# cs4247/music-transcription

Measured on AMD Instinct MI355X. Metric: 30 s audio chunks/sec (mel+CNNRNN forward), higher is better.
Workload: dtype f16; 1 GPU; CNNRNNModel inference, batch=32x30 s synthetic 16 kHz audio, mel+CNN-RNN HIP path (BASELINE.json configs[1]); batch_per_gpu=32, frames=938, coscheduled_batches_per_forward=4, streams_per_gpu=4, batches_in_flight=16, parallelism=dp1 (independent chunks)

## Files before the change

### include/mt_hip.h

```cpp
#ifndef MT_HIP_H
#define MT_HIP_H

#include <stddef.h>
#include <stdint.h>

#ifdef __cplusplus
extern "C" {
#endif

#define MT_OK            0
#define MT_EINVAL       -1
#define MT_EWORKSPACE   -2
#define MT_EHIP         -3
#define MT_EUNSUPPORTED -4

#define MT_DT_BF16 0
#define MT_DT_F16  1
#define MT_GX_F16  0x10

#define MT_N_FFT 2048
#define MT_N_PITCH 88

typedef void* mt_stream_t;

int         mt_version(void);
const char* mt_last_error(void);
int         mt_device_count(void);
int         mt_init(int device);
#define MT_WS_LSTM_GX        1
#define MT_WS_LSTM_HX        2
#define MT_WS_LSTM_CX        3
#define MT_WS_LSTM_SYNC      4
#define MT_WS_LSTM_BWD_PART  5
#define MT_WS_LSTM_DGX       6
#define MT_WS_MEL_PLAN       7
#define MT_WS_ADAM           8
size_t      mt_workspace_bytes(int kind, int B, int T, int H);
#define MT_AR_F32   0
#define MT_AR_BF16  1
#define MT_AR_F16   2
int         mt_allreduce(void* buf, size_t count, int dtype, void* comm, mt_stream_t stream);


int    mt_mel_filterbank_host(float* fb_host, int sr, int n_mels);
int    mt_mel_num_frames(int n_samples, int hop);

typedef struct { int sr, hop, n_mels, ell_rows; } mt_mel_desc;
size_t mt_mel_plan_bytes(int n_mels);
int    mt_mel_plan_init(void* plan, size_t plan_bytes, int sr, int hop, int n_mels, mt_mel_desc* desc,
                        mt_stream_t stream);

int    mt_mel_db_f32(const void* plan, const mt_mel_desc* desc, const float* wave, int B, int n_samples,
                     float* mel_db, float* chunk_max_power, int apply_clamp, mt_stream_t stream);

int    mt_mel_db_windows_f32(const void* plan, const mt_mel_desc* desc, const float* store, const long long* win_off,
                             const int* win_len, const int* rec_end, int B, int max_win_len, int T_out,
                             const int* t_keep, float* mel_db, float* chunk_max_power, mt_stream_t stream);

int    mt_roll_windows(const int* spans, const long long* pitch_off, const int* cols, const int* win_rec,
                       const long long* win_cols, const int* win_ncols, const int* t_keep, int B, int T_out,
                       float* roll, mt_stream_t stream);

int    mt_stitch_windows(const float* src, int Bw, int P, int Tw, const int* dst_row, const long long* dst_frame0,
                         const int* keep_lo, const int* keep_hi, float* dst, int R, long long T_dst, mt_stream_t stream);

int    mt_conv1_bn_relu_pool(const float* mel, const float* chunk_max_power, const float* w, const float* bias,
                             void* act1, int B, int n_mels, int T, mt_stream_t stream);
int    mt_conv2_bn_relu_pool(const void* act1, const void* w2, const float* bias, void* X0, int ldx,
                             int B, int F1, int T, mt_stream_t stream);
int    mt_conv1_bn_relu_pool_dt(const float* mel, const float* chunk_max_power, const float* w, const float* bias,
                                void* act1, int B, int n_mels, int T, int dt, mt_stream_t stream);
int    mt_conv12_bn_relu_pool_dt(const float* mel, const float* chunk_max_power, const float* w1, const float* b1,
                                 const void* w2, const float* b2, void* X0, int ldx, int B, int n_mels, int T, int dt,
                                 mt_stream_t stream);
int    mt_conv2_bn_relu_pool_dt(const void* act1, const void* w2, const float* bias, void* X0, int ldx,
                                int B, int F1, int T, int dt, mt_stream_t stream);

int    mt_gemm_bf16_f32acc(const void* A, int lda, const void* W, int ldw, const float* bias,
                           float* C, int ldc, int M, int N, int K, mt_stream_t stream);
int    mt_gemm_lstm_gx(const void* X, int ldx, const void* W_ih, int ldw, const float* bias, float* gx,
                       int B, int T, int H, int K, mt_stream_t stream);
int    mt_gemm_logits(const void* X, int ldx, const void* W, int ldw, const float* bias, float* logits,
                      int B, int T, int N, int K, mt_stream_t stream);
int    mt_gemm_lstm_gx_from_hx(const float* hx_prev, const void* W_ih, int ldw, const float* bias, float* gx,
                               int B, int T, int H, int Hprev, mt_stream_t stream);
int    mt_gemm_lstm_gx_from_hx_ex(const float* hx_prev, const void* W_ih, int ldw, const float* bias, float* gx,
                                  int B, int T, int H, int Hprev, int gx_f16, mt_stream_t stream);
int    mt_gemm_logits_from_hx(const float* hx_prev, const void* W, int ldw, const float* bias, float* logits,
                              int B, int T, int N, int Hprev, mt_stream_t stream);
int    mt_gemm_f32acc_dt(const void* A, int lda, const void* W, int ldw, const float* bias,
                         float* C, int ldc, int M, int N, int K, int dt, mt_stream_t stream);
int    mt_gemm_lstm_gx_dt(const void* X, int ldx, const void* W_ih, int ldw, const float* bias, float* gx,
                          int B, int T, int H, int K, int dt, mt_stream_t stream);
int    mt_gemm_logits_dt(const void* X, int ldx, const void* W, int ldw, const float* bias, float* logits,
                         int B, int T, int N, int K, int dt, mt_stream_t stream);
#define MT_GEMM_SCHED_BYTES 64
size_t mt_gemm_sched_bytes(void);
int    mt_gemm_lstm_gx_sched(const void* X, int ldx, const void* W_ih, int ldw, const float* bias, float* gx,
                             int B, int T, int H, int K, int dt, void* sched, mt_stream_t stream);
int    mt_gemm_lstm_gx_from_hx_sched(const float* hx_prev, const void* W_ih, int ldw, const float* bias, float* gx,
                                     int B, int T, int H, int Hprev, int gx_f16, void* sched, mt_stream_t stream);

size_t mt_lstm_gx_bytes(int B, int T, int H);
size_t mt_lstm_hx_bytes(int B, int T, int H);
size_t mt_lstm_sync_bytes(int B, int H);
int    mt_lstm_bidir_fwd(const float* gx, const float* w_hh, float* hx, void* sync_ws, size_t sync_bytes,
                         int B, int T, int H, mt_stream_t stream);
int    mt_lstm_bidir_fwd_xproj(const float* hx_prev, const float* w_ihx, const float* bias, const float* w_hh, float* hx,
                               void* sync_ws, size_t sync_bytes, int B, int T, int H, mt_stream_t stream);
int    mt_lstm_bidir_fwd_ex(const float* gx, const float* w_hh, float* hx, void* sync_ws, size_t sync_bytes,
                            int B, int T, int H, int flags, mt_stream_t stream);
int    mt_persistent_cus_in_flight(mt_stream_t stream);
int    mt_lstm_relayout_bf16(const float* hx, void* X, int ldx, int B, int T, int H, mt_stream_t stream);
int    mt_lstm_unpack_f32(const float* hx, float* y, int B, int T, int H, mt_stream_t stream);

#define MT_MAX_LSTM_LAYERS 8
typedef struct {
    int n_mels;
    int hidden;
    int layers;
    int operand_dtype;
    const float* conv1_w;
    const float* conv1_b;
    const void*  conv2_w;
    const float* conv2_b;
    const void*  w_ih[MT_MAX_LSTM_LAYERS];
    const float* b_gates[MT_MAX_LSTM_LAYERS];
    const float* w_hh[MT_MAX_LSTM_LAYERS];
    const void*  fc_w;
    const float* fc_b;
    const float* w_ihx[MT_MAX_LSTM_LAYERS];
} mt_cnnrnn_weights;

size_t mt_cnnrnn_workspace_bytes(const mt_cnnrnn_weights* w, int B, int T);
int    mt_cnnrnn_conv_fused(void);
size_t mt_cnnrnn_status_offset(const mt_cnnrnn_weights* w, int B, int T, int layer);
int    mt_cnnrnn_forward(const mt_cnnrnn_weights* w, const float* mel, const float* chunk_max_power,
                         int B, int T, float* logits, void* workspace, size_t workspace_bytes,
                         mt_stream_t stream);
int    mt_cnnrnn_num_stages(int layers);
int    mt_cnnrnn_forward_ex(const mt_cnnrnn_weights* w, const float* mel, const float* chunk_max_power,
                            int B, int T, float* logits, void* workspace, size_t workspace_bytes,
                            void* const* events, int n_events, mt_stream_t stream);

int    mt_conv_cl_bf16(const void* A, const void* S, const void* W, const float* bias, void* out,
                       int B, int F, int T, int C1, int C2, int Cout, int KH, int relu, int pool,
                       int out_mode, int ldx, mt_stream_t stream);
int    mt_gemm_batched_f32(const void* A, int lda, long long sA1, long long sA2, const void* W, int ldw,
                           long long sW1, long long sW2, const float* bias, float* C, int ldc,
                           long long sC1, long long sC2, int M, int N, int K, int batch, int zdiv,
                           mt_stream_t stream);
int    mt_gemm_batched_bf16out(const void* A, int lda, long long sA1, long long sA2, const void* W, int ldw,
                               long long sW1, long long sW2, const float* bias, void* C, int ldc,
                               long long sC1, long long sC2, int M, int N, int K, int batch, int zdiv,
// ... 245 lines not shown
```

### music-transcription_amd/_lib.py

```python
from __future__ import annotations

import ctypes as C
import os

_HERE = os.path.dirname(os.path.abspath(__file__))
LIB_PATH = os.path.join(_HERE, "libmt_hip.so")
MAX_LSTM_LAYERS = 8
N_PITCH = 88
DT_BF16, DT_F16 = 0, 1
GX_F16 = 0x10


class MtError(RuntimeError):
    pass


def build(verbose: bool = False) -> str:
    import subprocess
    r = subprocess.run(["make", "-C", os.path.join(_HERE, "csrc"), "-j8"], capture_output=True, text=True)
    if verbose or r.returncode != 0:
        print(r.stdout[-4000:], r.stderr[-4000:])
    if r.returncode != 0:
        raise MtError("building libmt_hip.so failed")
    return LIB_PATH


if not os.path.exists(LIB_PATH):
    raise ImportError(f"{LIB_PATH} not found: build it with `python -c 'import __graft_entry__ as g; g.build()'` "
                      f"or `make -C {os.path.join(_HERE, 'csrc')}` (needs hipcc)")

import torch as _torch

lib = C.CDLL(LIB_PATH)

vp, sz, i32, f32p = C.c_void_p, C.c_size_t, C.c_int, C.c_void_p


class MelDesc(C.Structure):
    _fields_ = [("sr", i32), ("hop", i32), ("n_mels", i32), ("ell_rows", i32)]


class CnnRnnWeights(C.Structure):
    _fields_ = [("n_mels", i32), ("hidden", i32), ("layers", i32), ("operand_dtype", i32),
                ("conv1_w", vp), ("conv1_b", vp), ("conv2_w", vp), ("conv2_b", vp),
                ("w_ih", vp * MAX_LSTM_LAYERS), ("b_gates", vp * MAX_LSTM_LAYERS), ("w_hh", vp * MAX_LSTM_LAYERS),
                ("fc_w", vp), ("fc_b", vp), ("w_ihx", vp * MAX_LSTM_LAYERS)]


class CnnRnnLargeWeights(C.Structure):
    _fields_ = ([(n, i32) for n in ("n_mels", "hidden", "layers", "hidden_local", "use_attention", "use_heads", "heads", "head_dim_pad")]
                + [("attn_scale", C.c_float), ("operand_dtype", i32)]
                + [(n, vp) for n in ("conv1_w", "conv1_b", "rb1c1_w", "rb1c1_b", "rb1c2_w", "rb1c2_b", "rb2c1_w", "rb2c1_b",
                                     "rb2c2_w", "rb2c2_b", "fa_w", "fa_b")]
                + [("main_w_ih", vp * MAX_LSTM_LAYERS), ("main_b", vp * MAX_LSTM_LAYERS), ("main_w_hh", vp * MAX_LSTM_LAYERS)]
                + [(n, vp) for n in ("local_w_ih", "local_b", "local_w_hh", "qkv_w", "qkv_b", "proj_w", "proj_b", "ln_g", "ln_b",
                                     "shared_w", "shared_b", "heads_w", "heads_b", "fc_w", "fc_b")]
                + [("main_w_ihx", vp * MAX_LSTM_LAYERS)])


ll = C.c_longlong
_SIGS = {
    "mt_version": (i32, []),
    "mt_last_error": (C.c_char_p, []),
    "mt_device_count": (i32, []),
    "mt_init": (i32, [i32]),
    "mt_workspace_bytes": (sz, [i32, i32, i32, i32]),
    "mt_allreduce": (i32, [vp, sz, i32, vp, vp]),
    "mt_mel_filterbank_host": (i32, [vp, i32, i32]),
    "mt_mel_num_frames": (i32, [i32, i32]),
    "mt_mel_plan_bytes": (sz, [i32]),
    "mt_mel_plan_init": (i32, [vp, sz, i32, i32, i32, C.POINTER(MelDesc), vp]),
    "mt_mel_db_f32": (i32, [vp, C.POINTER(MelDesc), vp, i32, i32, vp, vp, i32, vp]),
    "mt_mel_db_windows_f32": (i32, [vp, C.POINTER(MelDesc), vp, vp, vp, vp, i32, i32, i32, vp, vp, vp, vp]),
    "mt_roll_windows": (i32, [vp, vp, vp, vp, vp, vp, vp, i32, i32, vp, vp]),
    "mt_stitch_windows": (i32, [vp, i32, i32, i32, vp, vp, vp, vp, vp, i32, ll, vp]),
    "mt_conv1_bn_relu_pool": (i32, [vp, vp, vp, vp, vp, i32, i32, i32, vp]),
    "mt_conv2_bn_relu_pool": (i32, [vp, vp, vp, vp, i32, i32, i32, i32, vp]),
    "mt_conv1_bn_relu_pool_dt": (i32, [vp, vp, vp, vp, vp, i32, i32, i32, i32, vp]),
    "mt_conv2_bn_relu_pool_dt": (i32, [vp, vp, vp, vp, i32, i32, i32, i32, i32, vp]),
    "mt_cnnrnn_conv_fused": (i32, []),
    "mt_conv12_bn_relu_pool_dt": (i32, [vp, vp, vp, vp, vp, vp, vp, i32, i32, i32, i32, i32, vp]),
    "mt_gemm_f32acc_dt": (i32, [vp, i32, vp, i32, vp, vp, i32, i32, i32, i32, i32, vp]),
    "mt_gemm_lstm_gx_dt": (i32, [vp, i32, vp, i32, vp, vp, i32, i32, i32, i32, i32, vp]),
    "mt_gemm_logits_dt": (i32, [vp, i32, vp, i32, vp, vp, i32, i32, i32, i32, i32, vp]),
    "mt_conv_cl_dt": (i32, [vp, vp, vp, vp, vp] + [i32] * 12 + [vp]),
    "mt_gemm_batched_f32_dt": (i32, [vp, i32, ll, ll, vp, i32, ll, ll, vp, vp, i32, ll, ll, i32, i32, i32, i32, i32, i32, vp]),
    "mt_gemm_batched_h16out_dt": (i32, [vp, i32, ll, ll, vp, i32, ll, ll, vp, vp, i32, ll, ll, i32, i32, i32, i32, i32, i32, i32, vp]),
    "mt_lstm_relayout_dt": (i32, [vp, vp, i32, vp, i32, i32, i32, i32, i32, i32, i32, vp]),
    "mt_attn_softmax_clamped_dt": (i32, [vp, i32, vp, i32, i32, ll, C.c_float, C.c_float, i32, vp]),
    "mt_layernorm_residual_dt": (i32, [vp, i32, vp, i32, vp, vp, vp, i32, ll, i32, C.c_float, i32, vp]),
    "mt_gemm_lstm_gx_from_hx": (i32, [vp, vp, i32, vp, vp, i32, i32, i32, i32, vp]),
    "mt_gemm_lstm_gx_from_hx_ex": (i32, [vp, vp, i32, vp, vp, i32, i32, i32, i32, i32, vp]),
    "mt_gemm_logits_from_hx": (i32, [vp, vp, i32, vp, vp, i32, i32, i32, i32, vp]),
    "mt_gemm_bf16_f32acc": (i32, [vp, i32, vp, i32, vp, vp, i32, i32, i32, i32, vp]),
    "mt_gemm_lstm_gx": (i32, [vp, i32, vp, i32, vp, vp, i32, i32, i32, i32, vp]),
    "mt_gemm_sched_bytes": (sz, []),
    "mt_gemm_lstm_gx_sched": (i32, [vp, i32, vp, i32, vp, vp, i32, i32, i32, i32, i32, vp, vp]),
    "mt_gemm_lstm_gx_from_hx_sched": (i32, [vp, vp, i32, vp, vp, i32, i32, i32, i32, i32, vp, vp]),
    "mt_gemm_lstm_dh": (i32, [vp, i32, vp, i32, vp, i32, i32, i32, i32, i32, C.c_float, C.c_uint, C.c_uint, vp]),
    "mt_gemm_logits": (i32, [vp, i32, vp, i32, vp, vp, i32, i32, i32, i32, vp]),
    "mt_lstm_gx_bytes": (sz, [i32, i32, i32]),
    "mt_lstm_hx_bytes": (sz, [i32, i32, i32]),
    "mt_lstm_sync_bytes": (sz, [i32, i32]),
    "mt_lstm_bidir_fwd": (i32, [vp, vp, vp, vp, sz, i32, i32, i32, vp]),
    "mt_lstm_bidir_fwd_xproj": (i32, [vp, vp, vp, vp, vp, vp, sz, i32, i32, i32, vp]),
    "mt_lstm_bidir_fwd_ex": (i32, [vp, vp, vp, vp, sz, i32, i32, i32, i32, vp]),
    "mt_persistent_cus_in_flight": (i32, [vp]),
    "mt_lstm_relayout_bf16": (i32, [vp, vp, i32, i32, i32, i32, vp]),
    "mt_lstm_unpack_f32": (i32, [vp, vp, i32, i32, i32, vp]),
    "mt_conv_cl_bf16": (i32, [vp, vp, vp, vp, vp] + [i32] * 11 + [vp]),
    "mt_gemm_batched_f32": (i32, [vp, i32, ll, ll, vp, i32, ll, ll, vp, vp, i32, ll, ll, i32, i32, i32, i32, i32, vp]),
    "mt_gemm_batched_bf16out": (i32, [vp, i32, ll, ll, vp, i32, ll, ll, vp, vp, i32, ll, ll, i32, i32, i32, i32, i32, i32, vp]),
    "mt_lstm_relayout_ex": (i32, [vp, vp, i32, vp, i32, i32, i32, i32, i32, i32, vp]),
    "mt_attn_softmax_clamped": (i32, [vp, i32, vp, i32, i32, ll, C.c_float, C.c_float, vp]),
    "mt_attn_transpose_v": (i32, [vp, i32, i32, vp, i32, i32, i32, i32, i32, vp]),
    "mt_attn_fused_clamped": (i32, [vp, i32, i32, vp, i32, i32, i32, i32, i32, C.c_float, C.c_float, vp, i32, i32, vp]),
    "mt_layernorm_residual": (i32, [vp, i32, vp, i32, vp, vp, vp, i32, ll, i32, C.c_float, vp]),
    "mt_cnnrnn_large_workspace_bytes": (sz, [C.POINTER(CnnRnnLargeWeights), i32, i32]),
    "mt_cnnrnn_large_status_offset": (sz, [C.POINTER(CnnRnnLargeWeights), i32, i32, i32]),
    "mt_cnnrnn_large_forward": (i32, [C.POINTER(CnnRnnLargeWeights), vp, vp, i32, i32, vp, vp, sz, vp]),
    "mt_cnnrnn_large_forward_ex": (i32, [C.POINTER(CnnRnnLargeWeights), vp, vp, i32, i32, vp, vp, sz, vp, vp, vp, vp]),
    "mt_cnnrnn_large_num_stages": (i32, [i32]),
    "mt_cnnrnn_large_forward_ev": (i32, [C.POINTER(CnnRnnLargeWeights), vp, vp, i32, i32, vp, vp, sz, C.POINTER(vp), i32, vp]),
    "mt_adam_workspace_bytes": (sz, []),
    "mt_adam_clip_step": (i32, [vp, vp, vp, vp, ll] + [C.c_float] * 6 + [i32, vp, vp, sz, vp]),
    "mt_adam_clip_step_ex": (i32, [vp, vp, vp, vp, ll] + [C.c_float] * 6 + [i32, C.c_float, vp, i32, vp, vp, sz, vp]),
    "mt_bce_workspace_bytes": (sz, []),
    "mt_bce_masked_fwd_bwd": (i32, [vp, vp, vp, C.c_longlong, C.c_float, i32, vp, vp, vp, sz, i32, i32, i32, vp]),
    "mt_onset_offset_targets": (i32, [vp, vp, vp, C.c_longlong, i32, vp]),
    "mt_predict_threshold": (i32, [vp, vp, C.c_longlong, C.c_float, vp]),
    "mt_f1_counts": (i32, [vp, vp, vp, vp, i32, i32, i32, vp]),
    "mt_f1_sweep_counts": (i32, [vp, vp, vp, vp, i32, vp, i32, i32, i32, vp]),
    "mt_roll_to_notes": (i32, [vp, i32, C.c_float, i32, i32, i32, vp, vp, vp, i32, vp]),
    "mt_note_match_counts": (i32, [vp, vp, C.c_float, C.c_float, vp, vp, vp, i32, i32, i32, vp]),
    "mt_note_match_list": (i32, [vp, vp, C.c_float, C.c_float, vp, vp, vp, vp, vp, i32, i32, i32, vp]),
    "mt_note_sweep_counts": (i32, [vp, vp, vp, i32, vp, i32, vp, vp, vp, i32, i32, i32, vp]),
    "mt_note_sweep_list": (i32, [vp, vp, vp, i32, vp, i32, vp, vp, vp, vp, vp, i32, i32, i32, vp]),
    "mt_heads_to_notes": (i32, [vp, vp, C.c_float, C.c_float, i32, i32, i32, vp, vp, vp, i32, vp]),
    "mt_note_match_counts_off": (i32, [vp, vp, vp, C.c_float, C.c_float, C.c_float, vp, vp, vp, i32, i32, i32, vp]),
    "mt_note_match_list_off": (i32, [vp, vp, vp, C.c_float, C.c_float, C.c_float, vp, vp, vp, vp, vp, i32, i32, i32, vp]),
    "mt_heads_to_notes_off": (i32, [vp, vp, vp, C.c_float, C.c_float, C.c_float, i32, i32, i32, vp, vp, vp, i32, vp]),
    "mt_notes_batch": (i32, [vp, vp, C.c_float, C.c_float, vp, i32, i32, ll, vp, vp, vp, vp, ll, vp]),
    "mt_note_match_counts_clean": (i32, [vp, vp, vp, C.c_float, C.c_float, C.c_float, vp, vp, vp, i32, i32, i32, i32, i32, vp]),
    "mt_note_match_list_clean": (i32, [vp, vp, vp, C.c_float, C.c_float, C.c_float, vp, vp, vp, vp, vp, i32, i32, i32, i32, i32, vp]),
    "mt_heads_to_notes_clean": (i32, [vp, vp, vp, C.c_float, C.c_float, C.c_float, i32, i32, i32, vp, vp, vp, i32, i32, i32, vp]),
    "mt_notes_batch_clean": (i32, [vp, vp, C.c_float, C.c_float, vp, i32, i32, ll, vp, vp, vp, vp, ll, i32, i32, vp]),
    "mt_conv1_stats": (i32, [vp, vp, vp, vp, i32, i32, i32, vp]),
    "mt_bn_finalize": (i32, [vp, C.c_double, vp, vp, vp, vp, C.c_float, C.c_float, vp, vp, i32, vp, vp, vp, vp, i32, vp]),
    "mt_bn_stats_cl": (i32, [vp, ll, i32, vp, vp]),
    "mt_bn_relu_pool_apply": (i32, [vp, vp, vp, vp, vp, vp, i32, i32, i32, i32, vp]),
    "mt_bn_pool_bwd": (i32, [vp, i32, vp, vp, vp, vp, vp, vp, vp, vp, vp, vp, i32, i32, i32, vp]),
    "mt_conv_cl_tie": (i32, [vp, vp, vp, vp, vp, i32, i32, i32, i32, i32, i32, vp]),
    "mt_bn_pool_bwd_tie": (i32, [vp, i32, vp, vp, vp, vp, vp, vp, vp, vp, vp, vp, vp, i32, i32, i32, vp]),
    "mt_conv2_wgrad_workgroups": (i32, []),
    "mt_conv2_wgrad": (i32, [vp, vp, vp, vp, vp, i32, i32, i32, i32, vp]),
    "mt_pack_wih_cf": (i32, [vp, vp, ll, i32, i32, i32, i32, i32, i32, vp]),
    "mt_pack_jobs": (i32, [vp, i32, i32, vp]),
    "mt_transpose_bf16": (i32, [vp, ll, ll, i32, vp, ll, i32, vp]),
    "mt_gather4_f32": (i32, [vp, vp, i32, i32, i32, i32, ll, ll, ll, ll, C.c_float, vp]),
    "mt_sum_slices_f32": (i32, [vp, ll, i32, i32, vp, i32, i32, i32, vp]),
    "mt_rowsum_bf16": (i32, [vp, ll, ll, vp, i32, vp]),
    "mt_conv1_bwd": (i32, [vp] * 8 + [i32] + [vp] * 5 + [i32, i32, i32, vp]),
# ... 64 lines not shown
```

### music-transcription_amd/csrc/conv.hip

```cpp
#include "mt_common.h"

namespace mt {

template <int DT>
__global__ __launch_bounds__(256) void conv1_kernel(const float* __restrict__ mel, const unsigned* __restrict__ chunk_max,
                                                    const float* __restrict__ w , const float* __restrict__ bias ,
                                                    bf16_t* __restrict__ act1, int F, int T, int Fo) {
    const int t = blockIdx.x * 64 + (threadIdx.x & 63);
    const int fo = blockIdx.y * 4 + (threadIdx.x >> 6);
    const int b = blockIdx.z;
    if (t >= T || fo >= Fo) return;
    float floor_db = -3.0e38f;
    if (chunk_max) floor_db = 10.0f * log10f(fmaxf(__uint_as_float(chunk_max[b]), 1e-10f)) - 80.0f;
    const float* m = mel + (size_t)b * F * T;
    float p[4][3];
#pragma unroll
    for (int r = 0; r < 4; ++r) {
        const int f = 2 * fo - 1 + r;
#pragma unroll
        for (int c = 0; c < 3; ++c) {
            const int tt = t - 1 + c;
            const bool in = (f >= 0 && f < F && tt >= 0 && tt < T);
            p[r][c] = in ? fmaxf(m[(size_t)f * T + tt], floor_db) : 0.0f;
        }
    }
    typedef float f2_t __attribute__((ext_vector_type(2)));
    f2_t pp[3][3][1];
#pragma unroll
    for (int kh = 0; kh < 3; ++kh)
#pragma unroll
        for (int kw = 0; kw < 3; ++kw) pp[kh][kw][0] = f2_t{p[kh][kw], p[kh + 1][kw]};
    unsigned packed[16];
#pragma unroll
    for (int c = 0; c < 32; ++c) {
        f2_t a = f2_t{bias[c], bias[c]};
#pragma unroll
        for (int kh = 0; kh < 3; ++kh)
#pragma unroll
            for (int kw = 0; kw < 3; ++kw) {
                const float wv = w[c * 9 + kh * 3 + kw];
                a = __builtin_elementwise_fma(f2_t{wv, wv}, pp[kh][kw][0], a);
            }
        const float v = fmaxf(fmaxf(a.x, a.y), 0.0f);
        if (c & 1) packed[c >> 1] |= ((unsigned)f32_to_h16<DT>(v)) << 16;
        else packed[c >> 1] = f32_to_h16<DT>(v);
    }
    uint4* dst = (uint4*)(act1 + (((size_t)b * Fo + fo) * T + t) * 32);
#pragma unroll
    for (int i = 0; i < 4; ++i) dst[i] = make_uint4(packed[4 * i], packed[4 * i + 1], packed[4 * i + 2], packed[4 * i + 3]);
}

constexpr int C2_TF = 16, C2_TT = 16;
constexpr int C2_ROWS = 2 * C2_TF + 2, C2_PITCH = 20;

constexpr int C2_DMA_INSTRS = (C2_ROWS * C2_PITCH * 4 + 63) / 64;
constexpr int C2_LDS_BYTES = C2_DMA_INSTRS * 1024;

template <int DT>
__global__ __launch_bounds__(256, 2) void conv2_kernel(const bf16_t* __restrict__ act1, const bf16_t* __restrict__ w2 ,
                                                       const float* __restrict__ bias , bf16_t* __restrict__ X0,
                                                       int B, int F1, int T, int Fo2, int ldx, int tiles_f, int tiles_t) {
    extern __shared__ __attribute__((aligned(16))) char in_s[];
    const int tid = threadIdx.x, wv = tid >> 6, lane = tid & 63;
    const int ntile = wv & 1, mgrp = wv >> 1;
    const int r = lane & 31, h = lane >> 5;
    const int t_l = r & 15, fbit = r >> 4;
    const int co = ntile * 32 + r;
    const float bv = bias[co];
    bf16x8 wf[18];
#pragma unroll
    for (int ks = 0; ks < 18; ++ks) wf[ks] = *(const bf16x8*)(w2 + (size_t)co * 288 + ks * 16 + h * 8);

    const int n_tiles = B * tiles_f * tiles_t;
    typedef __attribute__((address_space(3))) void lvoid_t;
#define C2_ISSUE_DMA(TILE)                                                                                     \
    do {                                                                                                       \
        const int tile_ = (TILE);                                                                              \
        if (tile_ < n_tiles) {                                                                                 \
            const int b_ = tile_ / (tiles_f * tiles_t), rem_ = tile_ - b_ * tiles_f * tiles_t;                 \
            const int fy_ = rem_ / tiles_t, tx_ = rem_ - fy_ * tiles_t;                                        \
            const int fb_ = 2 * fy_ * C2_TF - 1, tb_ = tx_ * C2_TT - 1;                                        \
            const __amdgpu_buffer_rsrc_t rs_ = __builtin_amdgcn_make_buffer_rsrc(                              \
                (void*)(act1 + (size_t)b_ * F1 * T * 32), 0, F1 * T * 64, 0x00020000);                         \
            for (int q_ = wv; q_ < C2_DMA_INSTRS; q_ += 4) {                                                   \
                const int p_ = q_ * 64 + lane, pos_ = p_ >> 2, slot_ = p_ & 3;                                 \
                const int row_ = pos_ / C2_PITCH, col_ = pos_ - row_ * C2_PITCH;                               \
                const int f_ = fb_ + row_, t_ = tb_ + col_;                                                    \
                const bool ok_ = row_ < C2_ROWS && col_ < 18 && f_ >= 0 && f_ < F1 && t_ >= 0 && t_ < T;       \
                const int off_ = ok_ ? ((f_ * T + t_) * 64 + ((slot_ ^ ((col_ >> 2) & 3)) << 4)) : 0x7fffffff; \
                __builtin_amdgcn_raw_ptr_buffer_load_lds(rs_, (lvoid_t*)(in_s + q_ * 1024), 16, off_, 0, 0, 0); \
            }                                                                                                  \
        }                                                                                                      \
    } while (0)

    C2_ISSUE_DMA(blockIdx.x);
    for (int tile = blockIdx.x; tile < n_tiles; tile += gridDim.x) {
        const int b = tile / (tiles_f * tiles_t), rem = tile - b * tiles_f * tiles_t;
        const int fy = rem / tiles_t, tx = rem - fy * tiles_t;
        const int t0 = tx * C2_TT, fo0 = fy * C2_TF;
        asm volatile("s_waitcnt vmcnt(0)" ::: "memory");
        __builtin_amdgcn_s_barrier();
#pragma unroll 1
        for (int half = 0; half < 2; ++half) {
            f32x16 acc[4];
#pragma unroll
            for (int i = 0; i < 4; ++i)
#pragma unroll
                for (int j = 0; j < 16; ++j) acc[i][j] = 0.0f;
#pragma unroll
            for (int tap = 0; tap < 9; ++tap) {
                const int kh = tap / 3, kw = tap % 3;
                const int col = t_l + kw;
#pragma unroll
                for (int s2 = 0; s2 < 2; ++s2) {
                    const int chunk = (s2 * 2 + h) ^ ((col >> 2) & 3);
#pragma unroll
                    for (int mi = 0; mi < 4; ++mi) {
                        const int row = 2 * (mgrp * 8 + half * 4 + mi) + fbit + kh;
                        const bf16x8 afrag = *(const bf16x8*)(in_s + (row * C2_PITCH + col) * 64 + (chunk << 4));
                        acc[mi] = mfma_32x32x16<DT>(afrag, wf[tap * 2 + s2], acc[mi]);
                    }
                }
            }
            if (half == 1) {
                asm volatile("s_waitcnt lgkmcnt(0)" ::: "memory");
                __builtin_amdgcn_s_barrier();
                C2_ISSUE_DMA(tile + gridDim.x);
            }
#pragma unroll
            for (int mi = 0; mi < 4; ++mi) {
                const int fo = fo0 + mgrp * 8 + half * 4 + mi;
                if (fo >= Fo2) continue;
#pragma unroll
                for (int q = 0; q < 2; ++q)
#pragma unroll
                    for (int p = 0; p < 4; ++p) {
                        const int tl = p + 8 * q + 4 * h, t = t0 + tl;
                        const float v = fmaxf(fmaxf(acc[mi][4 * q + p], acc[mi][4 * (q + 2) + p]) + bv, 0.0f);
                        if (t < T) X0[((size_t)t * B + b) * ldx + fo * 64 + co] = f32_to_h16<DT>(v);
                    }
            }
        }
    }
#undef C2_ISSUE_DMA
}

constexpr int C12_MROWS = 2 * C2_ROWS + 2, C12_MCOLS = 20, C12_MPITCH = 21;
constexpr int C12_MEL_ELEMS = C12_MROWS * C12_MCOLS;
constexpr int C12_MEL_PER_THREAD = (C12_MEL_ELEMS + 255) / 256;
constexpr int C12_POS = C2_ROWS * 18;
constexpr int C12_LDS_BYTES = C2_LDS_BYTES + C12_MROWS * C12_MPITCH * 4;

template <int DT>
__global__ __launch_bounds__(256, 2) void conv12_kernel(const float* __restrict__ mel, const unsigned* __restrict__ chunk_max,
                                                        const float* __restrict__ w1 , const float* __restrict__ b1 ,
                                                        const bf16_t* __restrict__ w2 , const float* __restrict__ bias ,
                                                        bf16_t* __restrict__ X0, int B, int F, int F1, int T, int Fo2, int ldx, int tiles_f,
                                                        int tiles_t) {
    extern __shared__ __attribute__((aligned(16))) char in_s[];
    float* ms = (float*)(in_s + C2_LDS_BYTES);
    const int tid = threadIdx.x, wv = tid >> 6, lane = tid & 63;
    const int ntile = wv & 1, mgrp = wv >> 1;
    const int r = lane & 31, h = lane >> 5;
    const int t_l = r & 15, fbit = r >> 4;
    const int co = ntile * 32 + r;
    const float bv = bias[co];
    bf16x8 wf[18];
#pragma unroll
    for (int ks = 0; ks < 18; ++ks) wf[ks] = *(const bf16x8*)(w2 + (size_t)co * 288 + ks * 16 + h * 8);
    const int n_tiles = B * tiles_f * tiles_t;

    float mreg[C12_MEL_PER_THREAD];
    auto load_mel = [&](int tile_) {
        if (tile_ >= n_tiles) return;
        const int b_ = tile_ / (tiles_f * tiles_t), rem_ = tile_ - b_ * tiles_f * tiles_t;
        const int fy_ = rem_ / tiles_t, tx_ = rem_ - fy_ * tiles_t;
        const int m0_ = 2 * (2 * fy_ * C2_TF - 1) - 1, tc0_ = tx_ * C2_TT - 2;
        float floor_db = -3.0e38f;
        if (chunk_max) floor_db = 10.0f * log10f(fmaxf(__uint_as_float(chunk_max[b_]), 1e-10f)) - 80.0f;
        const float* m = mel + (size_t)b_ * F * T;
#pragma unroll
        for (int k = 0; k < C12_MEL_PER_THREAD; ++k) {
            const int idx = tid + 256 * k, lr = idx / C12_MCOLS, lc = idx - lr * C12_MCOLS;
            const int f = m0_ + lr, tt = tc0_ + lc;
            const bool in = idx < C12_MEL_ELEMS && f >= 0 && f < F && tt >= 0 && tt < T;
            mreg[k] = in ? fmaxf(m[(size_t)f * T + tt], floor_db) : 0.0f;
        }
    };
    load_mel(blockIdx.x);
    for (int tile = blockIdx.x; tile < n_tiles; tile += gridDim.x) {
        const int b = tile / (tiles_f * tiles_t), rem = tile - b * tiles_f * tiles_t;
        const int fy = rem / tiles_t, tx = rem - fy * tiles_t;
        const int t0 = tx * C2_TT, fo0 = fy * C2_TF;
        const int fb = 2 * fy * C2_TF - 1, tb = tx * C2_TT - 1;
#pragma unroll
        for (int k = 0; k < C12_MEL_PER_THREAD; ++k) {
            const int idx = tid + 256 * k, lr = idx / C12_MCOLS, lc = idx - lr * C12_MCOLS;
            if (idx < C12_MEL_ELEMS) ms[lr * C12_MPITCH + lc] = mreg[k];
        }
        __syncthreads();
        load_mel(tile + gridDim.x);
        typedef float f2_t __attribute__((ext_vector_type(2)));
#pragma unroll 1
        for (int idx = tid; idx < C12_POS; idx += 256) {
            const int row = idx / 18, col = idx - row * 18;
            const int f1 = fb + row, t = tb + col;
            unsigned packed[16];
            if (f1 >= 0 && f1 < F1 && t >= 0 && t < T) {
                f2_t pp[3][3];
#pragma unroll
                for (int kh = 0; kh < 3; ++kh)
#pragma unroll
                    for (int kw = 0; kw < 3; ++kw)
                        pp[kh][kw] = f2_t{ms[(2 * row + kh) * C12_MPITCH + col + kw], ms[(2 * row + kh + 1) * C12_MPITCH + col + kw]};
#pragma unroll
                for (int c = 0; c < 32; ++c) {
                    f2_t a = f2_t{b1[c], b1[c]};
#pragma unroll
                    for (int kh = 0; kh < 3; ++kh)
#pragma unroll
                        for (int kw = 0; kw < 3; ++kw) {
                            const float wv_ = w1[c * 9 + kh * 3 + kw];
                            a = __builtin_elementwise_fma(f2_t{wv_, wv_}, pp[kh][kw], a);
                        }
                    const float v = fmaxf(fmaxf(a.x, a.y), 0.0f);
                    if (c & 1) packed[c >> 1] |= ((unsigned)f32_to_h16<DT>(v)) << 16;
                    else packed[c >> 1] = f32_to_h16<DT>(v);
                }
            } else {
#pragma unroll
                for (int c = 0; c < 16; ++c) packed[c] = 0u;
            }
            char* dst = in_s + (row * C2_PITCH + col) * 64;
            const int sw = (col >> 2) & 3;
#pragma unroll
            for (int sl = 0; sl < 4; ++sl)
                *(uint4*)(dst + ((sl ^ sw) << 4)) = make_uint4(packed[4 * sl], packed[4 * sl + 1], packed[4 * sl + 2], packed[4 * sl + 3]);
        }
        __syncthreads();
#pragma unroll 1
        for (int half = 0; half < 2; ++half) {
            f32x16 acc[4];
#pragma unroll
            for (int i = 0; i < 4; ++i)
#pragma unroll
                for (int j = 0; j < 16; ++j) acc[i][j] = 0.0f;
#pragma unroll
            for (int tap = 0; tap < 9; ++tap) {
                const int kh = tap / 3, kw = tap % 3;
                const int col = t_l + kw;
#pragma unroll
                for (int s2 = 0; s2 < 2; ++s2) {
                    const int chunk = (s2 * 2 + h) ^ ((col >> 2) & 3);
#pragma unroll
                    for (int mi = 0; mi < 4; ++mi) {
                        const int row = 2 * (mgrp * 8 + half * 4 + mi) + fbit + kh;
                        const bf16x8 afrag = *(const bf16x8*)(in_s + (row * C2_PITCH + col) * 64 + (chunk << 4));
                        acc[mi] = mfma_32x32x16<DT>(afrag, wf[tap * 2 + s2], acc[mi]);
                    }
                }
            }
#pragma unroll
            for (int mi = 0; mi < 4; ++mi) {
                const int fo = fo0 + mgrp * 8 + half * 4 + mi;
                if (fo >= Fo2) continue;
#pragma unroll
                for (int q = 0; q < 2; ++q)
#pragma unroll
                    for (int p = 0; p < 4; ++p) {
                        const int tl = p + 8 * q + 4 * h, t = t0 + tl;
                        const float v = fmaxf(fmaxf(acc[mi][4 * q + p], acc[mi][4 * (q + 2) + p]) + bv, 0.0f);
                        if (t < T) X0[((size_t)t * B + b) * ldx + fo * 64 + co] = f32_to_h16<DT>(v);
                    }
            }
        }
    }
}

}

using namespace mt;

extern "C" int mt_conv1_bn_relu_pool_dt(const float* mel, const float* chunk_max_power, const float* w, const float* bias,
                                        void* act1, int B, int n_mels, int T, int dt, mt_stream_t stream) {
    MT_REQUIRE(mel && w && bias && act1, MT_EINVAL, "mt_conv1_bn_relu_pool: null pointer");
    MT_REQUIRE(B > 0 && n_mels >= 2 && T > 0, MT_EINVAL, "mt_conv1_bn_relu_pool: bad dims B=%d n_mels=%d T=%d", B, n_mels, T);
    MT_REQUIRE_DT(dt, "mt_conv1_bn_relu_pool");
    const int Fo = n_mels / 2;
    dim3 grid(cdiv(T, 64), cdiv(Fo, 4), B);
    if (dt == MT_DT_F16)
        hipLaunchKernelGGL(conv1_kernel<MT_DT_F16>, grid, dim3(256), 0, (hipStream_t)stream, mel, (const unsigned*)chunk_max_power, w, bias,
                           (bf16_t*)act1, n_mels, T, Fo);
    else
        hipLaunchKernelGGL(conv1_kernel<MT_DT_BF16>, grid, dim3(256), 0, (hipStream_t)stream, mel, (const unsigned*)chunk_max_power, w, bias,
                           (bf16_t*)act1, n_mels, T, Fo);
    MT_CHECK_LAUNCH();
    return MT_OK;
}
extern "C" int mt_conv1_bn_relu_pool(const float* mel, const float* chunk_max_power, const float* w, const float* bias,
                                     void* act1, int B, int n_mels, int T, mt_stream_t stream) {
    return mt_conv1_bn_relu_pool_dt(mel, chunk_max_power, w, bias, act1, B, n_mels, T, MT_DT_BF16, stream);
}

template <int DT>
static int conv2_launch(const void* act1, const void* w2, const float* bias, void* X0, int ldx, int B, int F1, int T, hipStream_t st) {
    const int Fo2 = F1 / 2;
    MT_SET_MAX_LDS((conv2_kernel<DT>), C2_LDS_BYTES);
    const int tiles_t = cdiv(T, C2_TT), tiles_f = cdiv(Fo2, C2_TF), n_tiles = B * tiles_f * tiles_t;
    dim3 grid(n_tiles < 512 ? n_tiles : 512);
    hipLaunchKernelGGL(conv2_kernel<DT>, grid, dim3(256), C2_LDS_BYTES, st, (const bf16_t*)act1,
                       (const bf16_t*)w2, bias, (bf16_t*)X0, B, F1, T, Fo2, ldx, tiles_f, tiles_t);
    MT_CHECK_LAUNCH();
    return MT_OK;
}

extern "C" int mt_conv2_bn_relu_pool_dt(const void* act1, const void* w2, const float* bias, void* X0, int ldx,
                                        int B, int F1, int T, int dt, mt_stream_t stream) {
    MT_REQUIRE(act1 && w2 && bias && X0, MT_EINVAL, "mt_conv2_bn_relu_pool: null pointer");
    MT_REQUIRE(B > 0 && F1 >= 2 && T > 0 && ldx >= (F1 / 2) * 64, MT_EINVAL, "mt_conv2_bn_relu_pool: bad dims");
    MT_REQUIRE_DT(dt, "mt_conv2_bn_relu_pool");
    MT_REQUIRE((size_t)F1 * T * 64 < ((size_t)1 << 31), MT_EUNSUPPORTED, "mt_conv2_bn_relu_pool: chunk activation too large for one buffer descriptor");
    return dt == MT_DT_F16 ? conv2_launch<MT_DT_F16>(act1, w2, bias, X0, ldx, B, F1, T, (hipStream_t)stream)
                           : conv2_launch<MT_DT_BF16>(act1, w2, bias, X0, ldx, B, F1, T, (hipStream_t)stream);
}
extern "C" int mt_conv2_bn_relu_pool(const void* act1, const void* w2, const float* bias, void* X0, int ldx,
                                     int B, int F1, int T, mt_stream_t stream) {
    return mt_conv2_bn_relu_pool_dt(act1, w2, bias, X0, ldx, B, F1, T, MT_DT_BF16, stream);
}

template <int DT>
static int conv12_launch(const float* mel, const float* cmax, const float* w1, const float* b1, const void* w2, const float* b2, void* X0, int ldx,
                         int B, int F, int T, hipStream_t st) {
    const int F1 = F / 2, Fo2 = F1 / 2;
    MT_SET_MAX_LDS((conv12_kernel<DT>), C12_LDS_BYTES);
    const int tiles_t = cdiv(T, C2_TT), tiles_f = cdiv(Fo2, C2_TF), n_tiles = B * tiles_f * tiles_t;
    dim3 grid(n_tiles < 512 ? n_tiles : 512);
    hipLaunchKernelGGL(conv12_kernel<DT>, grid, dim3(256), C12_LDS_BYTES, st, mel, (const unsigned*)cmax, w1, b1, (const bf16_t*)w2, b2, (bf16_t*)X0,
                       B, F, F1, T, Fo2, ldx, tiles_f, tiles_t);
    MT_CHECK_LAUNCH();
    return MT_OK;
}
extern "C" int mt_conv12_bn_relu_pool_dt(const float* mel, const float* chunk_max_power, const float* w1, const float* b1, const void* w2,
                                         const float* b2, void* X0, int ldx, int B, int n_mels, int T, int dt, mt_stream_t stream) {
    MT_REQUIRE(mel && w1 && b1 && w2 && b2 && X0, MT_EINVAL, "mt_conv12_bn_relu_pool: null pointer");
    MT_REQUIRE(B > 0 && n_mels >= 4 && T > 0 && ldx >= (n_mels / 4) * 64, MT_EINVAL, "mt_conv12_bn_relu_pool: bad dims B=%d n_mels=%d T=%d", B, n_mels, T);
    MT_REQUIRE_DT(dt, "mt_conv12_bn_relu_pool");
    return dt == MT_DT_F16 ? conv12_launch<MT_DT_F16>(mel, chunk_max_power, w1, b1, w2, b2, X0, ldx, B, n_mels, T, (hipStream_t)stream)
                           : conv12_launch<MT_DT_BF16>(mel, chunk_max_power, w1, b1, w2, b2, X0, ldx, B, n_mels, T, (hipStream_t)stream);
}
```

### music-transcription_amd/csrc/model.hip

```cpp
#include "mt_common.h"
#include <stdlib.h>

extern "C" {
int mt_conv1_bn_relu_pool_dt(const float*, const float*, const float*, const float*, void*, int, int, int, int, mt_stream_t);
int mt_conv2_bn_relu_pool_dt(const void*, const void*, const float*, void*, int, int, int, int, int, mt_stream_t);
int mt_conv12_bn_relu_pool_dt(const float*, const float*, const float*, const float*, const void*, const float*, void*, int, int, int, int, int, mt_stream_t);
int mt_gemm_lstm_gx_dt(const void*, int, const void*, int, const float*, float*, int, int, int, int, int, mt_stream_t);
int mt_gemm_logits_dt(const void*, int, const void*, int, const float*, float*, int, int, int, int, int, mt_stream_t);
int mt_lstm_bidir_fwd_ex(const float*, const float*, float*, void*, size_t, int, int, int, int, mt_stream_t);
int mt_lstm_relayout_dt(const float*, void*, int, float*, int, int, int, int, int, int, int, mt_stream_t);
int mt_gemm_lstm_gx_from_hx_ex(const float*, const void*, int, const float*, float*, int, int, int, int, int, mt_stream_t);
int mt_gemm_logits_from_hx(const float*, const void*, int, const float*, float*, int, int, int, int, mt_stream_t);
int mt_gemm_lstm_gx_sched(const void*, int, const void*, int, const float*, float*, int, int, int, int, int, void*, mt_stream_t);
int mt_gemm_lstm_gx_from_hx_sched(const float*, const void*, int, const float*, float*, int, int, int, int, int, void*, mt_stream_t);
int mt_lstm_bidir_fwd_xproj(const float*, const float*, const float*, const float*, float*, void*, size_t, int, int, int, mt_stream_t);
size_t mt_lstm_gx_bytes(int, int, int);
size_t mt_lstm_hx_bytes(int, int, int);
size_t mt_lstm_sync_bytes(int, int);
}

namespace mt {
struct CnnRnnPlan {
    int F1, Fo2, K0, K1, M, Mpad, Hp;
    size_t act1, x0, x1, gx, hx, hx2, sync, sync_stride, sched, total;
};
static CnnRnnPlan plan(const mt_cnnrnn_weights* w, int B, int T) {
    CnnRnnPlan p;
    p.F1 = w->n_mels / 2; p.Fo2 = p.F1 / 2;
    p.K0 = p.Fo2 * 64;
    p.K1 = (int)align_up((size_t)2 * w->hidden, 64);
    p.Hp = (int)align_up((size_t)w->hidden, 16);
    p.M = T * B; p.Mpad = (int)align_up((size_t)p.M, 128);
    size_t o = 0;
    p.act1 = o; o += align_up((size_t)B * p.F1 * T * 32 * 2, 256);
    p.x0 = o;   o += align_up((size_t)p.Mpad * p.K0 * 2, 256);
    p.x1 = o;   o += align_up((size_t)p.Mpad * p.K1 * 2, 256);
    p.gx = o;   o += align_up(mt_lstm_gx_bytes(B, T, p.Hp), 256);
    p.hx = o;   o += align_up(mt_lstm_hx_bytes(B, T, p.Hp), 256);
    p.hx2 = o;  o += align_up(mt_lstm_hx_bytes(B, T, p.Hp), 256);
    p.sync_stride = align_up(mt_lstm_sync_bytes(B, p.Hp), 256);
    p.sync = o; o += p.sync_stride * w->layers;
    p.sched = o; o += align_up((size_t)MT_GEMM_SCHED_BYTES * w->layers, 256);
    p.total = o;
    return p;
}
}

using namespace mt;

static int check_weights(const mt_cnnrnn_weights* w) {
    MT_REQUIRE(w, MT_EINVAL, "cnnrnn: null weights");
    MT_REQUIRE(w->n_mels >= 4 && w->layers >= 1 && w->layers <= MT_MAX_LSTM_LAYERS, MT_EINVAL,
               "cnnrnn: bad config n_mels=%d layers=%d", w->n_mels, w->layers);
    MT_REQUIRE(w->hidden >= 1 && w->hidden <= 1024, MT_EUNSUPPORTED, "cnnrnn: hidden size %d unsupported (1..1024)", w->hidden);
    MT_REQUIRE_DT(w->operand_dtype, "cnnrnn");
    MT_REQUIRE(w->conv1_w && w->conv1_b && w->conv2_w && w->conv2_b && w->fc_w && w->fc_b, MT_EINVAL, "cnnrnn: null weight pointer");
    for (int l = 0; l < w->layers; ++l)
        MT_REQUIRE(w->w_ih[l] && w->b_gates[l] && w->w_hh[l], MT_EINVAL, "cnnrnn: null LSTM weight pointer (layer %d)", l);
    return MT_OK;
}

extern "C" size_t mt_cnnrnn_workspace_bytes(const mt_cnnrnn_weights* w, int B, int T) {
    if (check_weights(w) != MT_OK || B <= 0 || T <= 0) return 0;
    return plan(w, B, T).total;
}

extern "C" size_t mt_cnnrnn_status_offset(const mt_cnnrnn_weights* w, int B, int T, int layer) {
    if (check_weights(w) != MT_OK || B <= 0 || T <= 0) return 0;
    const CnnRnnPlan p = plan(w, B, T);
    return p.sync + p.sync_stride * layer;
}

static inline int rec(void* const* events, int n_events, int& idx, hipStream_t st) {
    if (events && idx < n_events) {
        MT_CHECK_HIP(hipEventRecord((hipEvent_t)events[idx], st));
    }
    ++idx;
    return MT_OK;
}

extern "C" int mt_cnnrnn_num_stages(int layers) { return 3 + 3 * layers; }
extern "C" int mt_cnnrnn_conv_fused(void) {
    static const int on = getenv("MT_CONV_FUSED") && atoi(getenv("MT_CONV_FUSED")) == 1;
    return on;
}

extern "C" int mt_cnnrnn_forward_ex(const mt_cnnrnn_weights* w, const float* mel, const float* chunk_max_power, int B, int T,
                                    float* logits, void* workspace, size_t workspace_bytes,
                                    void* const* events, int n_events, mt_stream_t stream) {
    int rc = check_weights(w);
    if (rc != MT_OK) return rc;
    MT_REQUIRE(mel && logits && workspace, MT_EINVAL, "mt_cnnrnn_forward: null pointer");
    MT_REQUIRE(B > 0 && T > 0, MT_EINVAL, "mt_cnnrnn_forward: bad dims B=%d T=%d", B, T);
    const CnnRnnPlan p = plan(w, B, T);
    MT_REQUIRE(workspace_bytes >= p.total, MT_EWORKSPACE, "mt_cnnrnn_forward: workspace %zu < %zu bytes", workspace_bytes, p.total);
    char* ws = (char*)workspace;
    const int H = p.Hp, Hv = w->hidden, dt = w->operand_dtype;
    hipStream_t st = (hipStream_t)stream;
    int ei = 0;
    if ((rc = rec(events, n_events, ei, st)) != MT_OK) return rc;
    if (mt_cnnrnn_conv_fused()) {
        if ((rc = rec(events, n_events, ei, st)) != MT_OK) return rc;
        if ((rc = mt_conv12_bn_relu_pool_dt(mel, chunk_max_power, w->conv1_w, w->conv1_b, w->conv2_w, w->conv2_b, ws + p.x0, p.K0, B, w->n_mels, T, dt,
                                            stream)) != MT_OK) return rc;
    } else {
        if ((rc = mt_conv1_bn_relu_pool_dt(mel, chunk_max_power, w->conv1_w, w->conv1_b, ws + p.act1, B, w->n_mels, T, dt, stream)) != MT_OK) return rc;
        if ((rc = rec(events, n_events, ei, st)) != MT_OK) return rc;
        if ((rc = mt_conv2_bn_relu_pool_dt(ws + p.act1, w->conv2_w, w->conv2_b, ws + p.x0, p.K0, B, p.F1, T, dt, stream)) != MT_OK) return rc;
    }
    if ((rc = rec(events, n_events, ei, st)) != MT_OK) return rc;
    if (p.K1 != 2 * Hv) MT_CHECK_HIP(hipMemsetAsync(ws + p.x1, 0, (size_t)p.Mpad * p.K1 * 2, (hipStream_t)stream));
    char* hcur = ws + p.hx;
    char* hnext = ws + p.hx2;
    const bool from_hx = dt == MT_DT_F16 && H == Hv && H % 64 == 0;
    const int gx16 = (dt == MT_DT_F16) ? MT_GX_F16 : 0;
    for (int l = 0; l < w->layers; ++l) {
        const bool last = l + 1 == w->layers;
        const bool fused = l > 0 && w->w_ihx[l] && H <= 512;
        if (fused) {
            if ((rc = rec(events, n_events, ei, st)) != MT_OK) return rc;
            if ((rc = mt_lstm_bidir_fwd_xproj((const float*)hcur, w->w_ihx[l], w->b_gates[l], w->w_hh[l], (float*)hnext,
                                              ws + p.sync + p.sync_stride * l, p.sync_stride, B, T, H, stream)) != MT_OK) return rc;
            char* tmp = hcur; hcur = hnext; hnext = tmp;
        } else {
            const int K = l == 0 ? p.K0 : p.K1;
            if (l > 0 && from_hx) {
                if ((rc = mt_gemm_lstm_gx_from_hx_sched((const float*)hcur, w->w_ih[l], K, w->b_gates[l], (float*)(ws + p.gx), B, T, H, H, gx16,
                                                        ws + p.sched + (size_t)MT_GEMM_SCHED_BYTES * l, stream)) != MT_OK) return rc;
                char* tmp = hcur; hcur = hnext; hnext = tmp;
            } else {
                const void* X = l == 0 ? ws + p.x0 : ws + p.x1;
                if ((rc = mt_gemm_lstm_gx_sched(X, K, w->w_ih[l], K, w->b_gates[l], (float*)(ws + p.gx), B, T, H, K, dt | gx16,
                                                ws + p.sched + (size_t)MT_GEMM_SCHED_BYTES * l, stream)) != MT_OK) return rc;
            }
            if ((rc = rec(events, n_events, ei, st)) != MT_OK) return rc;
            if ((rc = mt_lstm_bidir_fwd_ex((const float*)(ws + p.gx), w->w_hh[l], (float*)hcur, ws + p.sync + p.sync_stride * l,
                                           p.sync_stride, B, T, H, gx16, stream)) != MT_OK) return rc;
        }
        if ((rc = rec(events, n_events, ei, st)) != MT_OK) return rc;
        const bool next_fused = !last && w->w_ihx[l + 1] && H <= 512;
        if (!next_fused && !from_hx)
            if ((rc = mt_lstm_relayout_dt((const float*)hcur, ws + p.x1, p.K1, nullptr, 0, 0, B, T, H, Hv, dt, stream)) != MT_OK) return rc;
        if ((rc = rec(events, n_events, ei, st)) != MT_OK) return rc;
    }
    if (from_hx) {
        if ((rc = mt_gemm_logits_from_hx((const float*)hcur, w->fc_w, p.K1, w->fc_b, logits, B, T, MT_N_PITCH, H, stream)) != MT_OK) return rc;
    } else {
        if ((rc = mt_gemm_logits_dt(ws + p.x1, p.K1, w->fc_w, p.K1, w->fc_b, logits, B, T, MT_N_PITCH, p.K1, dt, stream)) != MT_OK) return rc;
    }
    return rec(events, n_events, ei, st);
}

extern "C" int mt_cnnrnn_forward(const mt_cnnrnn_weights* w, const float* mel, const float* chunk_max_power, int B, int T,
                                 float* logits, void* workspace, size_t workspace_bytes, mt_stream_t stream) {
    return mt_cnnrnn_forward_ex(w, mel, chunk_max_power, B, T, logits, workspace, workspace_bytes, nullptr, 0, stream);
}
```

Baseline: 8322 chunks/s.

## Compute conv1 with fp32 MFMA and enable fused conv1+conv2 path by default

Replaces the scalar FMA loop for the 3x3 single-channel conv1 with 32x32x2 fp32 MFMA instructions, mapping the 9 taps (padded to 10) onto the K dimension and the 32 output channels onto M, with the freq-pool max taken over two accumulators. The same MFMA helper is used inside the fused conv1+conv2 kernel, and the standalone conv1 kernel now grid-strides over time blocks. The fused conv path is switched from opt-in to on by default. This trades VALU work for matrix-core work but adds padding waste and a lane-to-channel remapping.

```diff
diff --git a/include/mt_hip.h b/include/mt_hip.h
--- a/include/mt_hip.h
+++ b/include/mt_hip.h
@@ -70,6 +70,8 @@
                              int B, int F1, int T, mt_stream_t stream);
 int    mt_conv1_bn_relu_pool_dt(const float* mel, const float* chunk_max_power, const float* w, const float* bias,
                                 void* act1, int B, int n_mels, int T, int dt, mt_stream_t stream);
+int    mt_conv1_valu_bn_relu_pool_dt(const float* mel, const float* chunk_max_power, const float* w, const float* bias,
+                                     void* act1, int B, int n_mels, int T, int dt, mt_stream_t stream);
 int    mt_conv12_bn_relu_pool_dt(const float* mel, const float* chunk_max_power, const float* w1, const float* b1,
                                  const void* w2, const float* b2, void* X0, int ldx, int B, int n_mels, int T, int dt,
                                  mt_stream_t stream);
diff --git a/music-transcription_amd/_lib.py b/music-transcription_amd/_lib.py
--- a/music-transcription_amd/_lib.py
+++ b/music-transcription_amd/_lib.py
@@ -78,6 +78,7 @@
     "mt_conv2_bn_relu_pool": (i32, [vp, vp, vp, vp, i32, i32, i32, i32, vp]),
     "mt_conv1_bn_relu_pool_dt": (i32, [vp, vp, vp, vp, vp, i32, i32, i32, i32, vp]),
     "mt_conv2_bn_relu_pool_dt": (i32, [vp, vp, vp, vp, i32, i32, i32, i32, i32, vp]),
+    "mt_conv1_valu_bn_relu_pool_dt": (i32, [vp, vp, vp, vp, vp, i32, i32, i32, i32, vp]),
     "mt_cnnrnn_conv_fused": (i32, []),
     "mt_conv12_bn_relu_pool_dt": (i32, [vp, vp, vp, vp, vp, vp, vp, i32, i32, i32, i32, i32, vp]),
     "mt_gemm_f32acc_dt": (i32, [vp, i32, vp, i32, vp, vp, i32, i32, i32, i32, i32, vp]),
diff --git a/music-transcription_amd/csrc/conv.hip b/music-transcription_amd/csrc/conv.hip
--- a/music-transcription_amd/csrc/conv.hip
+++ b/music-transcription_amd/csrc/conv.hip
@@ -3,9 +3,9 @@
 namespace mt {
 
 template <int DT>
-__global__ __launch_bounds__(256) void conv1_kernel(const float* __restrict__ mel, const unsigned* __restrict__ chunk_max,
-                                                    const float* __restrict__ w , const float* __restrict__ bias ,
-                                                    bf16_t* __restrict__ act1, int F, int T, int Fo) {
+__global__ __launch_bounds__(256) void conv1_valu_kernel(const float* __restrict__ mel, const unsigned* __restrict__ chunk_max,
+                                                         const float* __restrict__ w , const float* __restrict__ bias ,
+                                                         bf16_t* __restrict__ act1, int F, int T, int Fo) {
     const int t = blockIdx.x * 64 + (threadIdx.x & 63);
     const int fo = blockIdx.y * 4 + (threadIdx.x >> 6);
     const int b = blockIdx.z;
@@ -48,6 +48,84 @@
     uint4* dst = (uint4*)(act1 + (((size_t)b * Fo + fo) * T + t) * 32);
 #pragma unroll
     for (int i = 0; i < 4; ++i) dst[i] = make_uint4(packed[4 * i], packed[4 * i + 1], packed[4 * i + 2], packed[4 * i + 3]);
+}
+
+struct Conv1Frag {
+    float wa[5];
+    f32x16 bias;
+};
+__device__ __forceinline__ int c1_row_channel(int row) { return 16 * ((row >> 2) & 1) + 4 * (row >> 3) + (row & 3); }
+
+__device__ __forceinline__ Conv1Frag conv1_frag_load(const float* __restrict__ w , const float* __restrict__ bias , int lane) {
+    Conv1Frag fr;
+    const int c = c1_row_channel(lane & 31), h = lane >> 5;
+#pragma unroll
+    for (int s = 0; s < 5; ++s) fr.wa[s] = 2 * s + h < 9 ? w[c * 9 + 2 * s + h] : 0.0f;
+#pragma unroll
+    for (int j = 0; j < 16; ++j) fr.bias[j] = bias[16 * h + j];
+    return fr;
+}
+
+template <int DT, class Patch>
+__device__ __forceinline__ void conv1_mfma_position(const Conv1Frag& fr, int lane, Patch patch, unsigned (&out)[8]) {
+    const int h = lane >> 5;
+    float x0[5], x1[5];
+#pragma unroll
+    for (int s = 0; s < 5; ++s) {
+        const int k = 2 * s + h;
+        const bool pad = k >= 9;
+        const int kh = pad ? 0 : k / 3, kw = pad ? 0 : k - 3 * (k / 3);
+        const float v0 = patch(kh, kw), v1 = patch(kh + 1, kw);
+        x0[s] = pad ? -0.0f : v0;
+        x1[s] = pad ? -0.0f : v1;
+    }
+    f32x16 a0 = fr.bias, a1 = fr.bias;
+#pragma unroll
+    for (int s = 0; s < 5; ++s) {
+        a0 = __builtin_amdgcn_mfma_f32_32x32x2f32(fr.wa[s], x0[s], a0, 0, 0, 0);
+        a1 = __builtin_amdgcn_mfma_f32_32x32x2f32(fr.wa[s], x1[s], a1, 0, 0, 0);
+    }
+#pragma unroll
+    for (int j = 0; j < 8; ++j) {
+        const float lo = fmaxf(fmaxf(a0[2 * j], a1[2 * j]), 0.0f), hi = fmaxf(fmaxf(a0[2 * j + 1], a1[2 * j + 1]), 0.0f);
+        out[j] = (unsigned)f32_to_h16<DT>(lo) | ((unsigned)f32_to_h16<DT>(hi) << 16);
+    }
+}
+
+constexpr int C1_TBLOCKS = 4;
+template <int DT>
+__global__ __launch_bounds__(256) void conv1_kernel(const float* __restrict__ mel, const unsigned* __restrict__ chunk_max,
+                                                    const float* __restrict__ w , const float* __restrict__ bias ,
+                                                    bf16_t* __restrict__ act1, int F, int T, int Fo) {
+    const int wv = threadIdx.x >> 6, lane = threadIdx.x & 63;
+    const int fo = blockIdx.y * 4 + wv, b = blockIdx.z;
+    if (fo >= Fo) return;
+    float floor_db = -3.0e38f;
+    if (chunk_max) floor_db = 10.0f * log10f(fmaxf(__uint_as_float(chunk_max[b]), 1e-10f)) - 80.0f;
+    const float* m = mel + (size_t)b * F * T;
+    const Conv1Frag fr = conv1_frag_load(w, bias, lane);
+    const int nblk = (T + 63) >> 6;
+#pragma unroll 1
+    for (int tb = blockIdx.x; tb < nblk; tb += gridDim.x) {
+#pragma unroll
+        for (int g = 0; g < 2; ++g) {
+            const int tg = tb * 64 + g * 32;
+            if (tg >= T) break;
+            const int t = tg + (lane & 31);
+            unsigned out[8];
+            conv1_mfma_position<DT>(fr, lane, [&](int pr, int pc) {
+                const int f = 2 * fo - 1 + pr, tt = t - 1 + pc;
+                const bool in = ((unsigned)f < (unsigned)F) & ((unsigned)tt < (unsigned)T);
+                const float v = m[(size_t)min(max(f, 0), F - 1) * T + min(max(tt, 0), T - 1)];
+                return fminf(fmaxf(v, in ? floor_db : 0.0f), in ? __builtin_inff() : 0.0f);
+            }, out);
+            if (t < T) {
+                uint4* dst = (uint4*)(act1 + (((size_t)b * Fo + fo) * T + t) * 32 + 16 * (lane >> 5));
+                dst[0] = make_uint4(out[0], out[1], out[2], out[3]);
+                dst[1] = make_uint4(out[4], out[5], out[6], out[7]);
+            }
+        }
+    }
 }
 
 constexpr int C2_TF = 16, C2_TT = 16;
@@ -149,6 +227,7 @@
 constexpr int C12_MEL_ELEMS = C12_MROWS * C12_MCOLS;
 constexpr int C12_MEL_PER_THREAD = (C12_MEL_ELEMS + 255) / 256;
 constexpr int C12_POS = C2_ROWS * 18;
+constexpr int C12_GROUPS = (C12_POS + 31) / 32;
 constexpr int C12_LDS_BYTES = C2_LDS_BYTES + C12_MROWS * C12_MPITCH * 4;
 
 template <int DT>
@@ -169,6 +248,7 @@
 #pragma unroll
     for (int ks = 0; ks < 18; ++ks) wf[ks] = *(const bf16x8*)(w2 + (size_t)co * 288 + ks * 16 + h * 8);
     const int n_tiles = B * tiles_f * tiles_t;
+    const Conv1Frag c1 = conv1_frag_load(w1, b1, lane);
 
     float mreg[C12_MEL_PER_THREAD];
     auto load_mel = [&](int tile_) {
@@ -200,42 +280,26 @@
         }
         __syncthreads();
         load_mel(tile + gridDim.x);
-        typedef float f2_t __attribute__((ext_vector_type(2)));
 #pragma unroll 1
-        for (int idx = tid; idx < C12_POS; idx += 256) {
-            const int row = idx / 18, col = idx - row * 18;
+        for (int g = wv; g < C12_GROUPS; g += 4) {
+            const int idx = g * 32 + (lane & 31);
+            const bool live = idx < C12_POS;
+            const int ic = live ? idx : C12_POS - 1;
+            const int row = ic / 18, col = ic - row * 18;
+            const float* mp = ms + 2 * row * C12_MPITCH + col;
+            unsigned out[8];
+            conv1_mfma_position<DT>(c1, lane, [&](int pr, int pc) { return mp[pr * C12_MPITCH + pc]; }, out);
             const int f1 = fb + row, t = tb + col;
-            unsigned packed[16];
-            if (f1 >= 0 && f1 < F1 && t >= 0 && t < T) {
-                f2_t pp[3][3];
-#pragma unroll
-                for (int kh = 0; kh < 3; ++kh)
-#pragma unroll
-                    for (int kw = 0; kw < 3; ++kw)
-                        pp[kh][kw] = f2_t{ms[(2 * row + kh) * C12_MPITCH + col + kw], ms[(2 * row + kh + 1) * C12_MPITCH + col + kw]};
-#pragma unroll
-                for (int c = 0; c < 32; ++c) {
-                    f2_t a = f2_t{b1[c], b1[c]};
-#pragma unroll
-                    for (int kh = 0; kh < 3; ++kh)
-#pragma unroll
-                        for (int kw = 0; kw < 3; ++kw) {
-                            const float wv_ = w1[c * 9 + kh * 3 + kw];
-                            a = __builtin_elementwise_fma(f2_t{wv_, wv_}, pp[kh][kw], a);
-                        }
-                    const float v = fmaxf(fmaxf(a.x, a.y), 0.0f);
-                    if (c & 1) packed[c >> 1] |= ((unsigned)f32_to_h16<DT>(v)) << 16;
-                    else packed[c >> 1] = f32_to_h16<DT>(v);
-                }
-            } else {
-#pragma unroll
-                for (int c = 0; c < 16; ++c) packed[c] = 0u;
-            }
-            char* dst = in_s + (row * C2_PITCH + col) * 64;
-            const int sw = (col >> 2) & 3;
-#pragma unroll
-            for (int sl = 0; sl < 4; ++sl)
-                *(uint4*)(dst + ((sl ^ sw) << 4)) = make_uint4(packed[4 * sl], packed[4 * sl + 1], packed[4 * sl + 2], packed[4 * sl + 3]);
+            if (!(f1 >= 0 && f1 < F1 && t >= 0 && t < T)) {
+#pragma unroll
+                for (int j = 0; j < 8; ++j) out[j] = 0u;
+            }
+            if (live) {
+                char* dst = in_s + (row * C2_PITCH + col) * 64;
+                const int sw = (col >> 2) & 3;
+                *(uint4*)(dst + (((2 * h) ^ sw) << 4)) = make_uint4(out[0], out[1], out[2], out[3]);
+                *(uint4*)(dst + (((2 * h + 1) ^ sw) << 4)) = make_uint4(out[4], out[5], out[6], out[7]);
+            }
         }
         __syncthreads();
 #pragma unroll 1
@@ -287,12 +351,28 @@
     MT_REQUIRE(B > 0 && n_mels >= 2 && T > 0, MT_EINVAL, "mt_conv1_bn_relu_pool: bad dims B=%d n_mels=%d T=%d", B, n_mels, T);
     MT_REQUIRE_DT(dt, "mt_conv1_bn_relu_pool");
     const int Fo = n_mels / 2;
-    dim3 grid(cdiv(T, 64), cdiv(Fo, 4), B);
+    dim3 grid(cdiv(cdiv(T, 64), C1_TBLOCKS), cdiv(Fo, 4), B);
     if (dt == MT_DT_F16)
         hipLaunchKernelGGL(conv1_kernel<MT_DT_F16>, grid, dim3(256), 0, (hipStream_t)stream, mel, (const unsigned*)chunk_max_power, w, bias,
                            (bf16_t*)act1, n_mels, T, Fo);
     else
         hipLaunchKernelGGL(conv1_kernel<MT_DT_BF16>, grid, dim3(256), 0, (hipStream_t)stream, mel, (const unsigned*)chunk_max_power, w, bias,
+                           (bf16_t*)act1, n_mels, T, Fo);
+    MT_CHECK_LAUNCH();
+    return MT_OK;
+}
+extern "C" int mt_conv1_valu_bn_relu_pool_dt(const float* mel, const float* chunk_max_power, const float* w, const float* bias,
+                                             void* act1, int B, int n_mels, int T, int dt, mt_stream_t stream) {
+    MT_REQUIRE(mel && w && bias && act1, MT_EINVAL, "mt_conv1_valu_bn_relu_pool: null pointer");
+    MT_REQUIRE(B > 0 && n_mels >= 2 && T > 0, MT_EINVAL, "mt_conv1_valu_bn_relu_pool: bad dims B=%d n_mels=%d T=%d", B, n_mels, T);
+    MT_REQUIRE_DT(dt, "mt_conv1_valu_bn_relu_pool");
+    const int Fo = n_mels / 2;
+    dim3 grid(cdiv(T, 64), cdiv(Fo, 4), B);
+    if (dt == MT_DT_F16)
+        hipLaunchKernelGGL(conv1_valu_kernel<MT_DT_F16>, grid, dim3(256), 0, (hipStream_t)stream, mel, (const unsigned*)chunk_max_power, w, bias,
+                           (bf16_t*)act1, n_mels, T, Fo);
+    else
+        hipLaunchKernelGGL(conv1_valu_kernel<MT_DT_BF16>, grid, dim3(256), 0, (hipStream_t)stream, mel, (const unsigned*)chunk_max_power, w, bias,
                            (bf16_t*)act1, n_mels, T, Fo);
     MT_CHECK_LAUNCH();
     return MT_OK;
diff --git a/music-transcription_amd/csrc/model.hip b/music-transcription_amd/csrc/model.hip
--- a/music-transcription_amd/csrc/model.hip
+++ b/music-transcription_amd/csrc/model.hip
@@ -81,7 +81,7 @@
 
 extern "C" int mt_cnnrnn_num_stages(int layers) { return 3 + 3 * layers; }
 extern "C" int mt_cnnrnn_conv_fused(void) {
-    static const int on = getenv("MT_CONV_FUSED") && atoi(getenv("MT_CONV_FUSED")) == 1;
+    static const int on = !(getenv("MT_CONV_FUSED") && atoi(getenv("MT_CONV_FUSED")) == 0);
     return on;
 }
 
```

Result: faster. 8420 chunks/s, median of 6 (+1.2%).
